# KC-decoder/Multimodal-Brain-Pattern-Identification_XAI

Measured on AMD Instinct MI355X. Metric: samples/sec train (multimodal SpectrogramCNN+EEGNet fusion, B=64/GPU, 4x128x256 spectro + 10000x19 EEG), higher is better.
Workload: dtype bf16

## Files before the change

include/brainxai.h:

```cpp
#ifndef BRAINXAI_H
#define BRAINXAI_H

#include <stddef.h>
#include <stdint.h>

#ifdef __cplusplus
extern "C" {
#endif

#define BX_VERSION 100

enum { BX_F32 = 0, BX_BF16 = 1 };
enum { BX_POOL_MAX = 0, BX_POOL_AVG = 1 };
enum { BX_OK = 0, BX_EINVAL = -1, BX_EDTYPE = -2, BX_EALIGN = -3, BX_EWORKSPACE = -4, BX_EHIP = -5,
       BX_EUNSUPPORTED = -6 };
enum { BX_ALGO_AUTO = 0, BX_ALGO_DIRECT = 1, BX_ALGO_MFMA = 2 };
enum { BX_EPI_RELU = 1, BX_EPI_MASK_BITS = 2 };

typedef void* bxStream;

int bx_version(void);
const char* bx_last_error_string(void);

int bx_nchw_to_nhwc(const float* src, void* dst, int B, int C, int H, int W, int Cp, int dtype, bxStream stream);
int bx_nhwc_to_nchw(const void* src, float* dst, int B, int C, int H, int W, int Cs, int dtype, bxStream stream);

int bx_conv3x3_pack(const float* w_oihw, float* packed_f32, void* packed_mfma, int Cout, int Cin,
                    int I_p, int O_p, int transpose_flip, bxStream stream);
size_t bx_conv3x3_packed_mfma_bytes(int I_p, int O_p);
size_t bx_conv3x3_packed_split_bytes(int I_p, int O_p);
int bx_conv3x3_pack_split(const float* w_oihw, void* packed_split, int Cout, int Cin, int I_p, int O_p, int transpose_flip,
                          bxStream stream);
typedef struct {
  const void* w_oihw;
  void* packed_mfma;
  int Cout, Cin, I_p, O_p, transpose_flip, block_begin;
} bxPackJob;
int bx_conv3x3_pack_many(const bxPackJob* jobs_device, int njobs, int total_blocks, bxStream stream);
int bx_conv3x3_pack_many_layout(const bxPackJob* jobs_device, int njobs, int total_blocks, const float* src_nchw,
                                void* dst_nhwc_bf16, int B, int C, int H, int W, int Cp, bxStream stream);
int bx_conv3x3_pack_layout_ex(const bxPackJob* jobs_device, int njobs, int total_blocks, const float* src_nchw,
                              const float* const* src_slot, void* dst_nhwc_bf16, int B, int C, int H, int W, int Cp, bxStream stream);
int bx_conv3x3_pack_many_step(const bxPackJob* jobs_device, int njobs, int total_blocks, const float* src_nchw,
                              void* dst_nhwc_bf16, int B, int C, int H, int W, int Cp, uint64_t* state_a, uint64_t* out_a,
                              uint64_t* state_b, uint64_t* out_b, bxStream stream);
int bx_conv3x3_pair_supported(int C0_p, int C1, int C2, int dtype);
int bx_conv3x3_pair(const void* x, const void* packed1_mfma, const float* bias1, const void* packed2_mfma, const float* bias2,
                    void* y1, void* y2, unsigned char* mask1, unsigned char* mask2, int B, int H, int W, int C0_p, int C1, int C2,
                    int dtype, bxStream stream);
int bx_conv3x3(const void* x, const float* packed_f32, const void* packed_mfma, const float* bias,
               const void* relu_mask_src, const void* addend, void* y,
               int B, int H, int W, int Ci, int Co, int dtype, int flags, int algo, bxStream stream);
size_t bx_conv3x3_wgrad_workspace(int B, int H, int W, int Ci_p, int Co, int dtype, int algo);
int bx_conv3x3_wgrad(const void* x, const void* dz, float* dw_oihw, float* dbias, int B, int H, int W,
                     int Cin, int Ci_p, int Co, int dtype, int algo, void* workspace, size_t workspace_bytes,
                     bxStream stream);
typedef struct {
  const void* partial; float* dw; float* db;
  int nsplit, Cin, Co, ma, nb, ztiles, nfrag4, valid;
} bxWgradPending;
int bx_conv3x3_wgrad_chained(const void* x, const void* dz, float* dw_oihw, float* dbias, int B, int H, int W, int Cin,
                             int Ci_p, int Co, int dtype, int algo, void* workspace, size_t workspace_bytes,
                             bxWgradPending* pending, bxStream stream);
int bx_conv3x3_wgrad_finish(bxWgradPending* pending, bxStream stream);
int bx_conv3x3_carry(const void* x, const float* packed_f32, const void* packed_mfma, const float* bias,
                     const void* relu_mask_src, const void* addend, void* y, int B, int H, int W, int Ci, int Co,
                     int dtype, int flags, int algo, bxWgradPending* pending, bxStream stream);
size_t bx_conv3x3_bwd_fused_workspace(int B, int H, int W, int with_w1);
int bx_conv3x3_bwd_fused(const void* dz, const void* xl, const void* packed_flip, void* dzo, const void* x0, float* dw, float* db,
                         float* dw0, float* db0, int B, int H, int W, int Cin0, void* workspace, size_t workspace_bytes,
                         bxWgradPending* pending, bxStream stream);

int bx_profile_next_conv3(void* ev_start, void* ev_stop);

typedef struct {
  int B, H, W;
  int Cin_p;
  int C;
  int pool;
  int training;
  float eps, momentum;
  float dropout_p;
  uint32_t salt;
  int dtype;
  uint32_t* sync;
  void* route;
} bxTailDesc;
size_t bx_block_tail_route_bytes(const bxTailDesc* d);
#define BX_TAIL_SYNC_WORDS 8192
#define BX_TAIL_SYNC_FWD 0
#define BX_TAIL_SYNC_BWD 4096
size_t bx_block_tail_workspace(const bxTailDesc* d);
int bx_block_tail_fwd(const bxTailDesc* d, const void* y3, const void* x, const float* w1x1, int Cin,
                      const float* b1x1, const float* bn_weight, const float* bn_bias,
                      float* running_mean, float* running_var, int64_t* num_batches_tracked,
                      const uint64_t* seed, void* pooled, void* out, float* save_mean, float* save_invstd,
                      void* workspace, size_t workspace_bytes, bxStream stream);
int bx_set_tree_max_rows(int rows);
int bx_set_tail_fold(int mask);
int bx_block_conv3_tail_fwd(const bxTailDesc* d, const void* y2, const void* w3_mfma, const float* b3, void* y3,
                            const void* x, const float* w1x1, int Cin, const float* b1x1, const float* bn_weight,
                            const float* bn_bias, float* running_mean, float* running_var, int64_t* num_batches_tracked,
                            const uint64_t* seed, void* pooled, void* out, float* save_mean, float* save_invstd,
                            void* workspace, size_t workspace_bytes, bxStream stream);
int bx_block_tail_bwd(const bxTailDesc* d, const void* dout, const void* y3, const void* x, const void* pooled,
                      const float* w1x1, int Cin, const float* bn_weight, const float* save_mean,
                      const float* save_invstd, const uint64_t* seed, void* dz3, void* dx_skip,
                      float* d_bn_weight, float* d_bn_bias, float* d_w1x1, float* d_b1x1,
                      void* workspace, size_t workspace_bytes, bxStream stream);
int bx_relu(const void* x, void* y, size_t n, int dtype, bxStream stream);

int bx_gap_fc_lsm_fwd(const void* feat, const float* w, const float* b, float* gap_out, float* logp,
                      int B, int HW, int C, int N, int dtype, bxStream stream);
int bx_gap_fc_lsm_bwd(const float* dlogp, const float* logp, const float* gap_out, const float* w,
                      void* dfeat, float* dw, float* db, int B, int HW, int C, int N, int dtype, bxStream stream);
int bx_linear_lsm_fwd(const float* x, const float* w, const float* b, float* logp, int B, int K, int N,
                      bxStream stream);
int bx_linear_lsm_bwd(const float* dlogp, const float* logp, const float* x, const float* w, float* dx,
                      float* dw, float* db, int B, int K, int N, bxStream stream);
int bx_fusion_head_fwd(const float* eeg_logp, const float* spec_logp, const float* w1, const float* b1,
                       const float* w2, const float* b2, float* hidden, float* logp, int B, int N, int Hd,
                       bxStream stream);
int bx_fusion_head_bwd(const float* dlogp, const float* logp, const float* hidden, const float* eeg_logp,
                       const float* spec_logp, const float* w1, const float* w2, float* d_eeg_logp,
// ... 151 lines not shown
```

multimodal-brain-pattern-identification_xai_amd/_lib.py:

```python
from __future__ import annotations

import ctypes as C
import os

HERE = os.path.dirname(os.path.abspath(__file__))
LIB_PATH = os.path.join(HERE, "libbrainxai.so")

BX_F32, BX_BF16 = 0, 1
BX_POOL_MAX, BX_POOL_AVG = 0, 1
BX_ALGO_AUTO, BX_ALGO_DIRECT, BX_ALGO_MFMA = 0, 1, 2
BX_EPI_RELU = 1
BX_EPI_MASK_BITS = 2
BX_TAIL_SYNC_WORDS = 8192
BX_EEG_CAM_CONV1, BX_EEG_CAM_DEPTHWISE, BX_EEG_CAM_SEPARABLE = 0, 1, 2

vp, i32, i64, u32, f32, sz = C.c_void_p, C.c_int, C.c_int64, C.c_uint32, C.c_float, C.c_size_t


class TailDesc(C.Structure):
    _fields_ = [("B", i32), ("H", i32), ("W", i32), ("Cin_p", i32), ("C", i32), ("pool", i32), ("training", i32),
                ("eps", f32), ("momentum", f32), ("dropout_p", f32), ("salt", u32), ("dtype", i32), ("sync", vp), ("route", vp)]


class EegDesc(C.Structure):
# ... 11 lines not shown
    _fields_ = [("B", i32), ("T2", i32), ("F2", i32), ("F3", i32), ("K3", i32), ("P3", i32), ("Hd", i32), ("N", i32), ("training", i32),
                ("eps", f32), ("momentum", f32), ("dropout_p", f32), ("salt", u32)]


class EegDeepParams(C.Structure):
    _fields_ = [(n, vp) for n in ("conv2_w", "bn4_w", "bn4_b", "bn4_rm", "bn4_rv", "bn4_nbt", "wq", "bq", "wk", "bk", "wv", "bv",
                                  "w1", "b1", "w2", "b2")]


class EegDeepGrads(C.Structure):
    _fields_ = [(n, vp) for n in ("conv2_w", "bn4_w", "bn4_b", "wq", "bq", "wk", "bk", "wv", "bv", "w1", "b1", "w2", "b2")]


class WgradPending(C.Structure):
    _fields_ = [("partial", vp), ("dw", vp), ("db", vp), ("nsplit", i32), ("Cin", i32), ("Co", i32), ("ma", i32), ("nb", i32),
                ("ztiles", i32), ("nfrag4", i32), ("valid", i32)]


class PackJob(C.Structure):
    _fields_ = [("w_oihw", vp), ("packed_mfma", vp), ("Cout", i32), ("Cin", i32), ("I_p", i32), ("O_p", i32),
                ("transpose_flip", i32), ("block_begin", i32)]


class EegGrads(C.Structure):
    _fields_ = [(n, vp) for n in ("conv1_w", "bn1_w", "bn1_b", "dw_w", "bn2_w", "bn2_b", "sep_w", "bn3_w", "bn3_b")]


P = C.POINTER
SIGNATURES = {
    "bx_version": (i32, []),
    "bx_last_error_string": (C.c_char_p, []),
    "bx_nchw_to_nhwc": (i32, [vp, vp, i32, i32, i32, i32, i32, i32, vp]),
    "bx_nhwc_to_nchw": (i32, [vp, vp, i32, i32, i32, i32, i32, i32, vp]),
    "bx_conv3x3_pack": (i32, [vp, vp, vp, i32, i32, i32, i32, i32, vp]),
    "bx_conv3x3_packed_mfma_bytes": (sz, [i32, i32]),
    "bx_conv3x3_packed_split_bytes": (sz, [i32, i32]),
    "bx_conv3x3_pack_split": (i32, [vp, vp, i32, i32, i32, i32, i32, vp]),
    "bx_conv3x3_pack_many": (i32, [vp, i32, i32, vp]),
    "bx_conv3x3_pack_many_layout": (i32, [vp, i32, i32, vp, vp, i32, i32, i32, i32, i32, vp]),
    "bx_conv3x3_pack_layout_ex": (i32, [vp, i32, i32, vp, vp, vp, i32, i32, i32, i32, i32, vp]),
    "bx_conv3x3_pair_supported": (i32, [i32, i32, i32, i32]),
    "bx_conv3x3_pair": (i32, [vp] * 9 + [i32] * 7 + [vp]),
    "bx_conv3x3_pack_many_step": (i32, [vp, i32, i32, vp, vp, i32, i32, i32, i32, i32, vp, vp, vp, vp, vp]),
    "bx_scale_dev": (i32, [vp, vp, vp, sz, vp]),
    "bx_abs": (i32, [vp, vp, sz, vp]),
    "bx_conv3x3": (i32, [vp, vp, vp, vp, vp, vp, vp, i32, i32, i32, i32, i32, i32, i32, i32, vp]),
    "bx_conv3x3_carry": (i32, [vp, vp, vp, vp, vp, vp, vp, i32, i32, i32, i32, i32, i32, i32, i32, P(WgradPending), vp]),
    "bx_conv3x3_wgrad_workspace": (sz, [i32, i32, i32, i32, i32, i32, i32]),
    "bx_conv3x3_wgrad": (i32, [vp, vp, vp, vp, i32, i32, i32, i32, i32, i32, i32, i32, vp, sz, vp]),
    "bx_conv3x3_wgrad_chained": (i32, [vp, vp, vp, vp, i32, i32, i32, i32, i32, i32, i32, i32, vp, sz, P(WgradPending), vp]),
    "bx_conv3x3_wgrad_finish": (i32, [P(WgradPending), vp]),
    "bx_conv3x3_bwd_fused_workspace": (sz, [i32, i32, i32, i32]),
    "bx_conv3x3_bwd_fused": (i32, [vp] * 9 + [i32] * 4 + [vp, sz, P(WgradPending), vp]),
    "bx_block_tail_workspace": (sz, [P(TailDesc)]),
    "bx_block_tail_fwd": (i32, [P(TailDesc), vp, vp, vp, i32, vp, vp, vp, vp, vp, vp, vp, vp, vp, vp, vp, vp, sz, vp]),
    "bx_set_tree_max_rows": (i32, [i32]),
    "bx_set_tail_fold": (i32, [i32]),
    "bx_block_tail_route_bytes": (sz, [vp]),
    "bx_block_conv3_tail_fwd": (i32, [P(TailDesc), vp, vp, vp, vp, vp, vp, i32, vp, vp, vp, vp, vp, vp, vp, vp, vp, vp, vp, vp, sz, vp]),
    "bx_block_tail_bwd": (i32, [P(TailDesc), vp, vp, vp, vp, vp, i32, vp, vp, vp, vp, vp, vp, vp, vp, vp, vp, vp, sz, vp]),
    "bx_relu": (i32, [vp, vp, sz, i32, vp]),
    "bx_gap_fc_lsm_fwd": (i32, [vp, vp, vp, vp, vp, i32, i32, i32, i32, i32, vp]),
    "bx_gap_fc_lsm_bwd": (i32, [vp, vp, vp, vp, vp, vp, vp, i32, i32, i32, i32, i32, vp]),
    "bx_linear_lsm_fwd": (i32, [vp, vp, vp, vp, i32, i32, i32, vp]),
    "bx_linear_lsm_bwd": (i32, [vp, vp, vp, vp, vp, vp, vp, i32, i32, i32, vp]),
    "bx_fusion_head_fwd": (i32, [vp, vp, vp, vp, vp, vp, vp, vp, i32, i32, i32, vp]),
    "bx_fusion_head_bwd": (i32, [vp] * 13 + [i32, i32, i32, vp]),
    "bx_mm_head_workspace": (sz, [i32, i32, i32]),
    "bx_mm_head_fwd": (i32, [vp] * 15 + [i32] * 7 + [vp]),
    "bx_mm_head_bwd": (i32, [vp] * 22 + [sz] + [i32] * 7 + [vp]),
    "bx_kldiv_fwd_bwd": (i32, [vp, vp, vp, vp, i32, i32, i32, f32, vp]),
    "bx_eeg_saved_bytes": (sz, [P(EegDesc)]),
    "bx_eeg_workspace": (sz, [P(EegDesc)]),
    "bx_eeg_features_fwd": (i32, [P(EegDesc), P(EegParams), vp, vp, vp, vp, vp, sz, vp]),
    "bx_eeg_features_bwd": (i32, [P(EegDesc), P(EegParams), vp, vp, vp, vp, P(EegGrads), vp, vp, sz, vp]),
    "bx_eeg_saved_layout": (i32, [P(EegDesc), P(sz), P(sz)]),
    "bx_eeg_gradcam_workspace": (sz, [P(EegDesc), i32, i32]),
    "bx_eeg_gradcam": (i32, [P(EegDesc), P(EegParams), vp, vp, vp, i32, i32, i32, vp, vp, vp, vp, sz, vp]),
    "bx_eeg_deep_saved_bytes": (sz, [P(EegDeepDesc)]),
    "bx_eeg_deep_workspace": (sz, [P(EegDeepDesc)]),
    "bx_eeg_deep_fwd": (i32, [P(EegDeepDesc), P(EegDeepParams), vp, vp, vp, vp, vp, vp, sz, vp]),
    "bx_eeg_deep_bwd": (i32, [P(EegDeepDesc), P(EegDeepParams), vp, vp, vp, vp, vp, P(EegDeepGrads), vp, vp, sz, vp]),
    "bx_attention_workspace": (sz, [i32]),
    "bx_attention_fwd": (i32, [vp] * 10 + [i32, i32, i32, vp]),
    "bx_attention_bwd": (i32, [vp] * 16 + [sz, i32, i32, i32, vp]),
    "bx_gradcam_reduce": (i32, [vp, vp, vp, vp, i32, i32, i32, i32, i32, i32, vp]),
    "bx_gradcam_head": (i32, [vp] * 12 + [i32] * 8 + [vp]),
    "bx_gradcam_head_sweep": (i32, [vp] * 4 + [i32] + [vp] * 8 + [i32] * 11 + [vp]),
    "bx_resize_bilinear": (i32, [vp, vp, i32, i32, i32, i32, i32, vp]),
    "bx_saliency_reduce": (i32, [vp, vp, i32, i32, i32, i32, f32, i32, vp]),
    "bx_axpby": (i32, [vp, vp, sz, f32, f32, vp]),
    "bx_mul": (i32, [vp, vp, vp, sz, vp]),
    "bx_ig_interpolate": (i32, [vp, vp, vp, vp, sz, i32, vp]),
    "bx_ig_accumulate": (i32, [vp, vp, vp, sz, i32, vp]),
    "bx_eeg_stack_iir": (i32, [vp, vp, vp, i32, i32, i32, i32, P(C.c_double), P(C.c_double), i32, i32, f32, f32, vp]),
    "bx_eeg_montage_workspace": (sz, [i32, i32, i32, i32]),
    "bx_eeg_montage_stack": (i32, [vp, vp, vp, vp, i32, i32, i32, i32, i32, P(C.c_double), P(C.c_double), i32, P(C.c_double), P(C.c_double),
                                   i32, f32, vp, vp, sz, vp]),
    "bx_spec_preprocess_workspace": (sz, [i32, i32, i32]),
    "bx_spec_preprocess": (i32, [vp, vp, vp, i32, i32, i32, i32, i32, i32, P(C.c_double), P(C.c_double), P(C.c_double), P(C.c_double),
                                 f32, vp, vp, sz, vp]),
    "bx_spec_regions_workspace": (sz, [i32]),
    "bx_spec_regions": (i32, [vp, vp, vp] + [i32] * 7 + [P(C.c_double), i32, P(C.c_double), i32, f32, vp, sz, vp]),
    "bx_adamw_step": (i32, [vp, vp, vp, vp, sz, f32, f32, f32, f32, f32, f32, vp, vp]),
    "bx_adamw_partials": (sz, [sz]),
    "bx_adamw_step_words": (sz, [sz]),
# ... 38 lines not shown
```

multimodal-brain-pattern-identification_xai_amd/csrc/conv3x3_mfma.hip:

```cpp
#include <stdlib.h>
#include "bx_common.h"
#include <string.h>

typedef __attribute__((ext_vector_type(8))) short bf16x8;
typedef __attribute__((ext_vector_type(4))) float f32x4;
typedef unsigned int u32x4 __attribute__((ext_vector_type(4)));
typedef unsigned int u32x2 __attribute__((ext_vector_type(2)));

static inline int mfma_ck(int Ci) { return Ci < 64 ? Ci : 64; }
static inline int mfma_ks(int ck) { return (9 * ck + 31) / 32; }

int bx_conv3x3_mfma_supported(int Ci, int Co, int dtype) {
  if (dtype != BX_BF16) return 0;
  if (!(Ci == 8 || Ci == 16 || Ci == 32 || (Ci >= 64 && Ci % 64 == 0))) return 0;
  return (Co >= 16 && Co % 16 == 0) || (Co == 8 && (Ci == 16 || Ci == 32));
}
static inline int mfma_ow(int O_p) { return O_p < 16 ? 16 : O_p; }
extern "C" size_t bx_conv3x3_packed_mfma_bytes(int I_p, int O_p) {
  if (!bx_conv3x3_mfma_supported(I_p, O_p, BX_BF16)) return 0;
  const int ck = mfma_ck(I_p);
  return (size_t)(I_p / ck) * mfma_ks(ck) * mfma_ow(O_p) * 32 * sizeof(bf16_t);
}

__global__ void k_pack_mfma(const float* __restrict__ w, bf16_t* __restrict__ wp, int Cout, int Cin, int I_p, int O_p, int tf,
// ... 2121 lines not shown
  constexpr int want_wgs = 512;
  const int want = want_wgs < p.ntiles ? want_wgs : p.ntiles;
  p.tps = (p.ntiles + want - 1) / want;
  p.nsplit = (p.ntiles + p.tps - 1) / p.tps;
  return p;
}
extern "C" size_t bx_conv3x3_bwd_fused_workspace(int B, int H, int W, int with_w1) {
  const FusedBwdPlan p = fused_bwd_plan(B, H, W);
  return (size_t)p.nsplit * (9 * 256 + 16) * sizeof(float) * (with_w1 ? 2 : 1);
}
extern "C" int bx_conv3x3_bwd_fused(const void* dz, const void* xl, const void* packed_flip, void* dzo, const void* x0, float* dw, float* db,
                                    float* dw0, float* db0, int B, int H, int W, int Cin0, void* ws, size_t ws_bytes, bxWgradPending* pending,
                                    bxStream stream) {
  hipStream_t s = (hipStream_t)stream;
  const bool w1 = x0 != nullptr;
  BX_REQUIRE(dz && xl && packed_flip && dw && db && ws && B > 0 && H > 0 && W > 0, "bx_conv3x3_bwd_fused: bad arguments");
  BX_REQUIRE(w1 ? (!dzo && dw0 && db0 && Cin0 > 0 && Cin0 <= 8) : (dzo && !dw0 && !db0),
             "bx_conv3x3_bwd_fused: either dzo (data gradient stored) or x0 with dw0 / db0 (conv1's weight gradient, 1..8 input channels)");
  BX_REQUIRE((size_t)B * H * W * 16 * 2 < ((size_t)1 << 31), "bx_conv3x3_bwd_fused: an activation tensor of 2 GiB or more is not supported");
  const FusedBwdPlan p = fused_bwd_plan(B, H, W);
  const size_t need = bx_conv3x3_bwd_fused_workspace(B, H, W, w1);
  BX_REQUIRE(ws_bytes >= need, "bx_conv3x3_bwd_fused: workspace %zu < %zu", ws_bytes, need);
  BX_REQUIRE(!pending || !pending->valid || pending->partial != ws, "bx_conv3x3_bwd_fused: the pending partials live in this call's workspace");
  WgradRedJob prev = {};
  int nred = 0;
  if (pending && pending->valid) { prev = wgrad_job_from(pending, true); nred = prev.nblocks; pending->valid = 0; }
  constexpr int IMG = 10 * 34 * 32;
  const size_t lds = w1 ? (size_t)3 * IMG + 8 * 32 * 32 : (size_t)2 * IMG;
  const uint32_t act_bytes = (uint32_t)((size_t)B * H * W * 16 * 2);
  float* part = (float*)ws;
  if (w1)
    hipLaunchKernelGGL((k_conv_mfma_bwd<true>), dim3((unsigned)(p.nsplit + nred)), dim3(256), lds, s, (const bf16_t*)dz, (const bf16_t*)xl,
                       (const bf16_t*)packed_flip, (const bf16_t*)x0, (bf16_t*)nullptr, part, H, W, p.tiles_x, p.tiles_y, p.ntiles, p.tps, p.nsplit,
                       act_bytes, prev, nred);
  else
    hipLaunchKernelGGL((k_conv_mfma_bwd<false>), dim3((unsigned)(p.nsplit + nred)), dim3(256), lds, s, (const bf16_t*)dz, (const bf16_t*)xl,
                       (const bf16_t*)packed_flip, (const bf16_t*)nullptr, (bf16_t*)dzo, part, H, W, p.tiles_x, p.tiles_y, p.ntiles, p.tps, p.nsplit,
                       act_bytes, prev, nred);
  BX_CHECK_LAUNCH("bx_conv3x3_bwd_fused");
  bxWgradPending cur = {};
  cur.partial = part; cur.dw = dw; cur.db = db; cur.nsplit = p.nsplit; cur.Cin = 16; cur.Co = 16; cur.ma = 1; cur.nb = 1;
  cur.ztiles = 1; cur.nfrag4 = 9 * 64; cur.valid = 1;
  if (!w1) {
    if (pending) { *pending = cur; return BX_OK; }
    return bx_wgrad_mfma_finish(&cur, s);
  }
  bxWgradPending cur0 = cur;
  cur0.partial = part + (size_t)p.nsplit * (9 * 256 + 16); cur0.dw = dw0; cur0.db = db0; cur0.Cin = Cin0;
  const WgradRedJob j1 = wgrad_job_from(&cur, false), j0 = wgrad_job_from(&cur0, false);
  hipLaunchKernelGGL(k_wgrad_reduce3, dim3((unsigned)(j1.nblocks + j0.nblocks)), dim3(256), 0, s, j1, j0);
  BX_CHECK_LAUNCH("bx_conv3x3_bwd_fused(reduce)");
  return BX_OK;
}
```

multimodal-brain-pattern-identification_xai_amd/ops.py:

```python
from __future__ import annotations

import ctypes as C
from types import SimpleNamespace

import torch

from . import _lib as L

CONV_ALGO = L.BX_ALGO_AUTO
WGRAD_ALGO = L.BX_ALGO_AUTO
CONV_PROFILE = None
import os as _os
OVERLAP_EEG = int(_os.environ.get("BX_OVERLAP_EEG", "1"))
OVERLAP_EEG_DDP = _os.environ.get("BX_OVERLAP_EEG_DDP", "0") == "1"


def overlap_eeg_now() -> bool:
    if CONV_PROFILE is not None or not (OVERLAP_EEG >= 2 or (OVERLAP_EEG == 1 and torch.cuda.is_current_stream_capturing())):
        return False
    import torch.distributed as dist
    return OVERLAP_EEG_DDP or not (dist.is_available() and dist.is_initialized())


def fork_eeg(device, *read_on_side):
# ... 387 lines not shown
def _wg_chain_state(device):
    key = device.index if device.index is not None else torch.cuda.current_device()
    st = _WG_CHAIN.get(key)
    if st is None:
        st = SimpleNamespace(pend=L.WgradPending(), ring=[None, None], slot=0, keep=None, stream=None, retired=[])
        _WG_CHAIN[key] = st
    return st


def wgrad_flush(device=None):
    for key, st in list(_WG_CHAIN.items()):
        if device is not None and key != (device.index if device.index is not None else torch.cuda.current_device()):
            continue
        if st.pend.valid:
            L.check(L.load().bx_conv3x3_wgrad_finish(C.byref(st.pend), st.stream), "bx_conv3x3_wgrad_finish")
        st.keep = None


def _wgrad(x, dz, w: torch.Tensor, b: torch.Tensor, chain: bool = False):
    lib = L.load()
    B, H, W, Cip = x.shape
    Co = dz.shape[3]
    dt = bx_dtype(x.dtype)
    algo = WGRAD_ALGO
    need = lib.bx_conv3x3_wgrad_workspace(B, H, W, Cip, Co, dt, algo)
    dw, db = new_grad(w), new_grad(b)
    if chain and WGRAD_CHAIN and algo != L.BX_ALGO_DIRECT:
        st = _wg_chain_state(x.device)
        if st.pend.valid and st.stream != _stream():
            wgrad_flush(x.device)
        buf = st.ring[st.slot]
        if buf is None or buf.numel() < need:
            if buf is not None:
                st.retired.append(buf)
            big = max([int(need), 1 << 20] + [b.numel() for b in st.ring if b is not None])
            buf = torch.empty(big, dtype=torch.uint8, device=x.device)
            st.ring[st.slot] = buf
        st.stream = _stream()
        with _Timed("wgrad", ("conv", B, H, W, Cip, Co)):
            L.check(lib.bx_conv3x3_wgrad_chained(_p(x), _p(dz), _p(dw), _p(db), B, H, W, w.shape[1], Cip, Co, dt, algo, _p(buf), buf.numel(),
                                                 C.byref(st.pend), st.stream), "bx_conv3x3_wgrad_chained")
        st.keep = (buf, dw, db)
        st.slot ^= 1
        return dw, db
    ws = workspace(need, x.device)
    with _Timed("wgrad", ("conv", B, H, W, Cip, Co)):
        L.check(lib.bx_conv3x3_wgrad(_p(x), _p(dz), _p(dw), _p(db), B, H, W, w.shape[1], Cip, Co, dt, algo, _p(ws), ws.numel(), _stream()),
                "bx_conv3x3_wgrad")
    return dw, db


def _bwd_fused(dz, xl, packed, w, b, x0, w0, b0):
    lib = L.load()
    B, H, W, _ = dz.shape
    st = _wg_chain_state(dz.device)
    if st.pend.valid and st.stream != _stream():
        wgrad_flush(dz.device)
    need = lib.bx_conv3x3_bwd_fused_workspace(B, H, W, 1 if x0 is not None else 0)
    buf = st.ring[st.slot]
    if buf is None or buf.numel() < need:
        if buf is not None:
            st.retired.append(buf)
        big = max([int(need), 1 << 20] + [t.numel() for t in st.ring if t is not None])
        buf = torch.empty(big, dtype=torch.uint8, device=dz.device)
        st.ring[st.slot] = buf
    st.stream = _stream()
    dw, db = new_grad(w), new_grad(b)
    dw0, db0 = (new_grad(w0), new_grad(b0)) if x0 is not None else (None, None)
    dzo = torch.empty_like(dz) if x0 is None else None
    if packed[1] is None or packed[4] != "bf16":
        raise RuntimeError("brainxai: the fused stage-1 backward needs the bf16 MFMA data-gradient operand")
    with _Timed("dgrad", ("conv", B, H, W, 16, 16)):
        L.check(lib.bx_conv3x3_bwd_fused(_p(dz), _p(xl), _p(packed[1]), _p(dzo), _p(x0), _p(dw), _p(db), _p(dw0), _p(db0), B, H, W,
                                         w0.shape[1], _p(buf), buf.numel(), C.byref(st.pend), st.stream), "bx_conv3x3_bwd_fused")
    if x0 is None:
        st.keep = (buf, dw, db)
        st.slot ^= 1
    else:
        st.keep = None
    return dw, db, dzo, (dw0, db0)


def _tail_desc(x, shape, dt, cfg, route=None) -> L.TailDesc:
    B, H, W, Cc = shape
    return L.TailDesc(B, H, W, x.shape[3], Cc, L.BX_POOL_MAX if cfg.pool == "max" else L.BX_POOL_AVG, 1 if cfg.training else 0,
                      cfg.eps, cfg.momentum, float(cfg.dropout_p), cfg.salt, bx_dtype(dt), _p(cfg.sync), _p(route))


class BlockFn(torch.autograd.Function):

    @staticmethod
    def forward(ctx, x, w1, b1, w2, b2, w3, b3, bnw, bnb, w11, b11, rm, rv, nbt, cfg):
        lib = L.load()
        dt = x.dtype
        ws_, bs_ = (w1, w2, w3), (b1, b2, b3)
        acts, pre = [x], None
        B, H, W, _ = x.shape
        Cc = w3.shape[0]
        fused = FUSE_POOL and dt == torch.bfloat16 and CONV_ALGO != L.BX_ALGO_DIRECT and cfg.preact != 3 and Cc >= 16
        packed3 = None
        first = 0
        masks = None
        fuse_bwd = False
        if (CONV_PAIR and dt == torch.bfloat16 and CONV_ALGO != L.BX_ALGO_DIRECT and cfg.preact not in (1, 2)
                and lib.bx_conv3x3_pair_supported(x.shape[3], w1.shape[0], w2.shape[0], bx_dtype(dt))):
            pk = []
            for k in range(2):
                packed = cfg.prepacked.get(cfg.pack_base + k, False) if cfg.prepacked is not None else None
                pk.append(packed if packed is not None else _pack(ws_[k], flip=False, dtype=dt))
            if pk[0][1] is not None and pk[1][1] is not None:
                need_y1 = cfg.keep is not None or (getattr(cfg, "grad_mode", True) and any(ctx.needs_input_grad[:11]))
                y1 = torch.empty(B, H, W, w1.shape[0], dtype=dt, device=x.device) if need_y1 else None
                y2 = torch.empty(B, H, W, w2.shape[0], dtype=dt, device=x.device)
                fuse_bwd = (need_y1 and cfg.keep is None and WGRAD_ALGO != L.BX_ALGO_DIRECT and x.shape[3] == 8
                            and tuple(w2.shape[:2]) == (16, 16) and tuple(w3.shape[:2]) == (16, 16) and any(ctx.needs_input_grad[1:11]))
                if need_y1 and MASK_BITS and w1.shape[0] <= 32 and not fuse_bwd:
                    masks = (torch.empty(B, H, W, w1.shape[0] // 4, dtype=torch.uint8, device=x.device),
                             torch.empty(B, H, W, w2.shape[0] // 4, dtype=torch.uint8, device=x.device))
                with _Timed("fwd", ("pair", B, H, W, x.shape[3], (w1.shape[0], w2.shape[0]))):
                    L.check(lib.bx_conv3x3_pair(_p(x), _p(pk[0][1]), _p(b1), _p(pk[1][1]), _p(b2), _p(y1), _p(y2),
                                                _p(masks[0]) if masks else None, _p(masks[1]) if masks else None, B, H, W, x.shape[3],
                                                w1.shape[0], w2.shape[0], bx_dtype(dt), _stream()), "bx_conv3x3_pair")
                acts += [y1 if y1 is not None else x.new_empty(0), y2]
                first = 2
        for k in range(first, 3):
            packed = cfg.prepacked.get(cfg.pack_base + k, False) if cfg.prepacked is not None else None
            if packed is None:
                packed = _pack(ws_[k], flip=False, dtype=dt)
            if k == 2 and fused and packed[1] is not None:
                packed3 = packed
                break
            if cfg.preact == k + 1:
                pre = _conv(acts[-1], packed, bs_[k], None, None, False, dt)
                y = torch.empty_like(pre)
                L.check(lib.bx_relu(_p(pre), _p(y), pre.numel(), bx_dtype(dt), _stream()), "bx_relu")
            else:
                y = _conv(acts[-1], packed, bs_[k], None, None, True, dt)
            acts.append(y)
        seed = None
        if cfg.training and cfg.dropout_p > 0:
            seed = cfg.seed if cfg.seed is not None else next_seed(x.device)
        pooled = torch.empty(B, H // 2, W // 2, Cc, dtype=dt, device=x.device)
        out = torch.empty_like(pooled)
        mean = torch.empty(Cc, dtype=torch.float32, device=x.device)
        invstd = torch.empty_like(mean)
        route = None
        if packed3 is not None:
            need_bwd = getattr(cfg, "grad_mode", True) and any(ctx.needs_input_grad[:11])
            use_route = TAIL_ROUTE and cfg.keep is None
            y3 = torch.empty(B, H, W, Cc, dtype=dt, device=x.device) if (cfg.keep is not None or (need_bwd and not use_route)) else None
            if need_bwd and use_route:
                route = torch.empty(B * (H // 2) * (W // 2) * Cc // 2, dtype=torch.uint8, device=x.device)
            desc = _tail_desc(x, (B, H, W, Cc), dt, cfg, route)
            ws = workspace(lib.bx_block_tail_workspace(C.byref(desc)), x.device)
            if CONV_PROFILE is not None:
                pe0, pe1 = torch.cuda.Event(enable_timing=True), torch.cuda.Event(enable_timing=True)
                pe0.record(); pe1.record()
                L.check(lib.bx_profile_next_conv3(pe0.cuda_event, pe1.cuda_event), "bx_profile_next_conv3")
                CONV_PROFILE.append(("fwd", pe0, pe1, ("conv3+pool", B, H, W, acts[2].shape[3], Cc)))
            L.check(lib.bx_block_conv3_tail_fwd(C.byref(desc), _p(acts[2]), _p(packed3[1]), _p(b3), _p(y3), _p(x), _p(w11), w11.shape[1], _p(b11),
                                                _p(bnw), _p(bnb), _p(rm), _p(rv), _p(nbt), _p(seed), _p(pooled), _p(out), _p(mean), _p(invstd),
                                                _p(ws), ws.numel(), _stream()), "bx_block_conv3_tail_fwd")
            acts.append(y3)
        else:
            y3 = acts[3]
            desc = _tail_desc(x, tuple(y3.shape), dt, cfg)
            ws = workspace(lib.bx_block_tail_workspace(C.byref(desc)), x.device)
            L.check(lib.bx_block_tail_fwd(C.byref(desc), _p(y3), _p(x), _p(w11), w11.shape[1], _p(b11), _p(bnw), _p(bnb), _p(rm), _p(rv), _p(nbt),
                                          _p(seed), _p(pooled), _p(out), _p(mean), _p(invstd), _p(ws), ws.numel(), _stream()), "bx_block_tail_fwd")
        ctx.cfg, ctx.desc, ctx.seed = cfg, desc, seed
        ctx.masks = masks
        ctx.fuse_bwd = fuse_bwd
        ctx.route, ctx.y3_shape = route, (B, H, W, Cc)
        ctx.save_for_backward(x, acts[1], acts[2], y3 if y3 is not None else x.new_empty(0), pooled, mean, invstd, w1, b1, w2, b2, w3, b3,
                              bnw, bnb, w11, b11)
        if pre is not None:
            cfg.capture["act"] = pre
        if cfg.keep is not None:
            cfg.keep["acts"] = (acts[1], acts[2], y3)
        return out

    @staticmethod
    def backward(ctx, dout):
        lib = L.load()
        x, y1, y2, y3, pooled, mean, invstd, w1, b1, w2, b2, w3, b3, bnw, bnb, w11, b11 = ctx.saved_tensors
        cfg, desc, seed = ctx.cfg, ctx.desc, ctx.seed
        dt = x.dtype
        need_dx = ctx.needs_input_grad[0]
        need_w = any(ctx.needs_input_grad[1:11])
        dout = dout.contiguous()
        dz3 = torch.empty(ctx.y3_shape, dtype=dt, device=x.device)
        if y3.numel() == 0:
            y3 = None
        dx_skip = torch.empty_like(x) if need_dx else None
        need_bn = ctx.needs_input_grad[7] or ctx.needs_input_grad[8]
        d_bnw, d_bnb = (new_grad(bnw), new_grad(bnb)) if need_bn else (torch.empty_like(bnw), torch.empty_like(bnb))
        d_w11, d_b11 = (new_grad(w11), new_grad(b11)) if need_w else (None, None)
        ws = workspace(lib.bx_block_tail_workspace(C.byref(desc)), x.device)
        L.check(lib.bx_block_tail_bwd(C.byref(desc), _p(dout), _p(y3), _p(x), _p(pooled), _p(w11), w11.shape[1], _p(bnw), _p(mean), _p(invstd),
                                      _p(seed), _p(dz3), _p(dx_skip), _p(d_bnw), _p(d_bnb), _p(d_w11), _p(d_b11), _p(ws), ws.numel(), _stream()),
                "bx_block_tail_bwd")
        if cfg.preact == 3:
            cfg.capture["grad"] = dz3
        acts = (x, y1, y2)
        wts = (w1, w2, w3)
        bss = (b1, b2, b3)
        grads_w, grads_b = [None] * 3, [None] * 3
        dz = dz3
        layers = (2, 1, 0)
        if ctx.fuse_bwd and need_w:
            for k in (2, 1):
                packed = cfg.prepacked.get(cfg.pack_base + k, True) if cfg.prepacked is not None else None
                w1_form = k == 1 and not need_dx
                grads_w[k], grads_b[k], dz, g0 = _bwd_fused(dz, acts[k], packed or _pack(wts[k], flip=True, dtype=dt), wts[k], bss[k],
                                                            x if w1_form else None, w1, b1)
            if w1_form:
                grads_w[0], grads_b[0] = g0
            layers = () if w1_form else (0,)
        for k in layers:
            if need_w:
                grads_w[k], grads_b[k] = _wgrad(acts[k], dz, wts[k], bss[k], chain=True)
            packed = cfg.prepacked.get(cfg.pack_base + k, True) if cfg.prepacked is not None else None
            if k > 0:
                mb = ctx.masks is not None and CONV_ALGO != L.BX_ALGO_DIRECT
                dz = _conv(dz, packed or _pack(wts[k], flip=True, dtype=dt), None, ctx.masks[k - 1] if mb else acts[k], None, False, dt,
                           mask_bits=mb)
                if cfg.preact == k:
                    cfg.capture["grad"] = dz
            elif need_dx:
                dz = _conv(dz, packed or _pack(wts[0], flip=True, dtype=dt), None, None, dx_skip, False, dt, carry=need_w)
        if need_w:
            wgrad_flush(x.device)
        dx = dz if need_dx else None
        if not need_bn:
            d_bnw = d_bnb = None
        return (dx, grads_w[0], grads_b[0], grads_w[1], grads_b[1], grads_w[2], grads_b[2], d_bnw, d_bnb, d_w11, d_b11,
                None, None, None, None)


class GapFcLsmFn(torch.autograd.Function):

    @staticmethod
    def forward(ctx, feat, w, b):
        B, H, W, Cc = feat.shape
        N = w.shape[0]
        gap = torch.empty(B, Cc, dtype=torch.float32, device=feat.device)
        logp = torch.empty(B, N, dtype=torch.float32, device=feat.device)
        L.check(L.load().bx_gap_fc_lsm_fwd(_p(feat), _p(w), _p(b), _p(gap), _p(logp), B, H * W, Cc, N, bx_dtype(feat.dtype), _stream()),
                "bx_gap_fc_lsm_fwd")
        ctx.shape, ctx.dt = (B, H, W, Cc), feat.dtype
        ctx.save_for_backward(gap, logp, w, b)
        return logp

    @staticmethod
    def backward(ctx, dlogp):
        gap, logp, w, b = ctx.saved_tensors
        B, H, W, Cc = ctx.shape
        N = w.shape[0]
        dfeat = torch.empty(B, H, W, Cc, dtype=ctx.dt, device=gap.device) if ctx.needs_input_grad[0] else None
        need_w = ctx.needs_input_grad[1] or ctx.needs_input_grad[2]
        dw, db = (new_grad(w), new_grad(b)) if need_w else (None, None)
        dlogp = dlogp.contiguous()
        L.check(L.load().bx_gap_fc_lsm_bwd(_p(dlogp), _p(logp), _p(gap), _p(w), _p(dfeat), _p(dw), _p(db), B, H * W, Cc, N,
                                           bx_dtype(ctx.dt), _stream()), "bx_gap_fc_lsm_bwd")
        return dfeat, dw, db

# ... 288 lines not shown
```

Baseline: 48380.

## Add fused dgrad+wgrad backward kernel for 32-channel conv3x3 stage

Adds an MFMA kernel that, for 32->32 conv3x3 layers, computes the data gradient (with ReLU masking from the saved activation) and accumulates the weight and bias gradient partials in the same pass over an LDS-staged tile. It also runs the previous layer's pending wgrad reduction in extra blocks. The Python path now routes the second-stage block (16->32->32->32, W>16) through this fused backward instead of separate dgrad and wgrad launches. This is meant to remove a second read of dz and activations plus launch overhead. In exchange the second stage no longer stores mask bits, and the kernel adds LDS and register pressure.

```diff
diff --git a/include/brainxai.h b/include/brainxai.h
--- a/include/brainxai.h
+++ b/include/brainxai.h
@@ -70,6 +70,9 @@
 int bx_conv3x3_bwd_fused(const void* dz, const void* xl, const void* packed_flip, void* dzo, const void* x0, float* dw, float* db,
                          float* dw0, float* db0, int B, int H, int W, int Cin0, void* workspace, size_t workspace_bytes,
                          bxWgradPending* pending, bxStream stream);
+size_t bx_conv3x3_bwd_fused32_workspace(int B, int H, int W);
+int bx_conv3x3_bwd_fused32(const void* dz, const void* xl, const void* packed_flip, void* dzo, float* dw, float* db, int B, int H, int W,
+                           int Cin, int Co, void* workspace, size_t workspace_bytes, bxWgradPending* pending, bxStream stream);
 
 int bx_profile_next_conv3(void* ev_start, void* ev_stop);
 
diff --git a/multimodal-brain-pattern-identification_xai_amd/_lib.py b/multimodal-brain-pattern-identification_xai_amd/_lib.py
--- a/multimodal-brain-pattern-identification_xai_amd/_lib.py
+++ b/multimodal-brain-pattern-identification_xai_amd/_lib.py
@@ -87,6 +87,8 @@
     "bx_conv3x3_wgrad_finish": (i32, [P(WgradPending), vp]),
     "bx_conv3x3_bwd_fused_workspace": (sz, [i32, i32, i32, i32]),
     "bx_conv3x3_bwd_fused": (i32, [vp] * 9 + [i32] * 4 + [vp, sz, P(WgradPending), vp]),
+    "bx_conv3x3_bwd_fused32_workspace": (sz, [i32, i32, i32]),
+    "bx_conv3x3_bwd_fused32": (i32, [vp] * 6 + [i32] * 5 + [vp, sz, P(WgradPending), vp]),
     "bx_block_tail_workspace": (sz, [P(TailDesc)]),
     "bx_block_tail_fwd": (i32, [P(TailDesc), vp, vp, vp, i32, vp, vp, vp, vp, vp, vp, vp, vp, vp, vp, vp, vp, sz, vp]),
     "bx_set_tree_max_rows": (i32, [i32]),
diff --git a/multimodal-brain-pattern-identification_xai_amd/csrc/conv3x3_mfma.hip b/multimodal-brain-pattern-identification_xai_amd/csrc/conv3x3_mfma.hip
--- a/multimodal-brain-pattern-identification_xai_amd/csrc/conv3x3_mfma.hip
+++ b/multimodal-brain-pattern-identification_xai_amd/csrc/conv3x3_mfma.hip
@@ -2197,3 +2197,209 @@
   BX_CHECK_LAUNCH("bx_conv3x3_bwd_fused(reduce)");
   return BX_OK;
 }
+
+__global__ __launch_bounds__(256, 2) void k_conv_mfma_bwd32(const bf16_t* __restrict__ dz, const bf16_t* __restrict__ xl, const bf16_t* __restrict__ wp,
+    bf16_t* __restrict__ dzo, float* __restrict__ partial, int H, int W, int tiles_x, int tiles_y, int ntiles, int tps, int nsplit,
+    uint32_t act_bytes, WgradRedJob red, int nred) {
+  constexpr int TH = 8, TW = 32, HWID = TW + 2, HH = TH + 2, RB = 64, KS = 9, MP = TH * TW / 64, TPR = TW / 16, NC = 2;
+  constexpr int NU = HH * HWID * 4, NR = (NU + 255) / 256;
+  constexpr int IMG = HH * HWID * RB;
+  constexpr int NT = 36, PER_SPLIT = NT * 256 + 32;
+  extern __shared__ __attribute__((aligned(16))) char lds[];
+  if ((int)blockIdx.x < nred) {
+    if ((int)blockIdx.x < red.nblocks) wgrad_reduce3_body(red, (int)blockIdx.x, reinterpret_cast<float4*>(lds));
+    return;
+  }
+  const int split = (int)blockIdx.x - nred;
+  char* xs = lds;
+  char* zs = lds + IMG;
+  const int wave = threadIdx.x >> 6, lane = threadIdx.x & 63, g = lane >> 4, li = lane & 15;
+  const int q = li >> 2, pc = li & 3;
+  const int m = wave >> 1, n = wave & 1;
+  const bool want_bias = m == 0;
+  const __amdgpu_buffer_rsrc_t zres = __builtin_amdgcn_make_buffer_rsrc((void*)dz, 0, act_bytes, 0x00020000);
+  const __amdgpu_buffer_rsrc_t xres = __builtin_amdgcn_make_buffer_rsrc((void*)xl, 0, act_bytes, 0x00020000);
+  const __amdgpu_buffer_rsrc_t yres = __builtin_amdgcn_make_buffer_rsrc((void*)dzo, 0, act_bytes, 0x00020000);
+  int hpy[NR], hpx[NR];
+  uint32_t hrel[NR];
+#pragma unroll
+  for (int k = 0; k < NR; ++k) {
+    const int u = threadIdx.x + k * 256;
+    const int p = u / 4, c = u % 4;
+    hpy[k] = u < NU ? p / HWID - 1 : -100000;
+    hpx[k] = p % HWID - 1;
+    hrel[k] = (uint32_t)(((p / HWID - 1) * W + (p % HWID - 1)) * 32 + c * 8) * 2u;
+  }
+  uint4 rz[NR], rx[NR];
+  auto fetch = [&](int tile) {
+    const int tx = tile % tiles_x, ty = (tile / tiles_x) % tiles_y, b = tile / (tiles_x * tiles_y);
+    const int y0 = ty * TH, xo = tx * TW;
+    const uint32_t pix0 = (uint32_t)((b * H + y0) * W + xo);
+#pragma unroll
+    for (int k = 0; k < NR; ++k) {
+      const bool ok = (unsigned)(y0 + hpy[k]) < (unsigned)H && (unsigned)(xo + hpx[k]) < (unsigned)W;
+      const uint32_t off = ok ? pix0 * 64u + hrel[k] : 0x80000000u;
+      const u32x4 v = __builtin_amdgcn_raw_buffer_load_b128(zres, off, 0, 0);
+      const u32x4 w = __builtin_amdgcn_raw_buffer_load_b128(xres, off, 0, 0);
+      rz[k] = make_uint4(v.x, v.y, v.z, v.w);
+      rx[k] = make_uint4(w.x, w.y, w.z, w.w);
+    }
+  };
+  int xbase[2], zbase[2];
+#pragma unroll
+  for (int h = 0; h < 2; ++h) {
+    const int c = 8 * g + 4 * h + q;
+    xbase[h] = c * RB + (((m ^ (c >> 3)) & 1) << 5) + pc * 8;
+    zbase[h] = (HWID + c + 1) * RB + (((n ^ ((c + 1) >> 2)) & 1) << 5) + pc * 8;
+  }
+  int xbase2;
+  {
+    const int c = 8 * g + q + 8;
+    xbase2 = c * RB + (((m ^ (c >> 3)) & 1) << 5) + pc * 8;
+  }
+  f32x4 aw[9];
+#pragma unroll
+  for (int t = 0; t < 9; ++t) aw[t] = (f32x4){0.f, 0.f, 0.f, 0.f};
+  float bsum = 0.f;
+  auto load_frags = [&](int ks, bf16x8 (&a)[9], bf16x8& bb) {
+    bb = tr_read8(zs, zbase[0] + ks * HWID * RB, zbase[1] + ks * HWID * RB);
+#pragma unroll
+    for (int dy = 0; dy < 3; ++dy) {
+      const int ro = (ks + dy) * HWID * RB;
+      const u32x2 p0 = __builtin_bit_cast(u32x2, __builtin_amdgcn_ds_read_tr16_b64_v4i16((lds_s16x4*)(xs + xbase[0] + ro)));
+      const u32x2 p1 = __builtin_bit_cast(u32x2, __builtin_amdgcn_ds_read_tr16_b64_v4i16((lds_s16x4*)(xs + xbase[1] + ro)));
+      const u32x2 p2 = __builtin_bit_cast(u32x2, __builtin_amdgcn_ds_read_tr16_b64_v4i16((lds_s16x4*)(xs + xbase2 + ro)));
+      const uint32_t d0 = p0.x, d1 = p0.y, d2 = p1.x, d3 = p1.y, d4 = p2.x;
+      a[dy * 3 + 0] = __builtin_bit_cast(bf16x8, (u32x4){d0, d1, d2, d3});
+      a[dy * 3 + 1] = __builtin_bit_cast(bf16x8, (u32x4){__builtin_amdgcn_alignbit(d1, d0, 16), __builtin_amdgcn_alignbit(d2, d1, 16),
+                                                         __builtin_amdgcn_alignbit(d3, d2, 16), __builtin_amdgcn_alignbit(d4, d3, 16)});
+      a[dy * 3 + 2] = __builtin_bit_cast(bf16x8, (u32x4){d1, d2, d3, d4});
+    }
+  };
+  auto mma = [&](const bf16x8 (&a)[9], const bf16x8& bb) {
+    if (want_bias) {
+#pragma unroll
+      for (int j = 0; j < 8; ++j) bsum += __uint_as_float(((uint32_t)(unsigned short)bb[j]) << 16);
+    }
+#pragma unroll
+    for (int tap = 0; tap < 9; ++tap) aw[tap] = __builtin_amdgcn_mfma_f32_16x16x32_bf16(a[tap], bb, aw[tap], 0, 0, 0);
+  };
+  const int t_begin = split * tps;
+  const int t_end = t_begin + tps < ntiles ? t_begin + tps : ntiles;
+  if (t_begin < t_end) fetch(t_begin);
+  for (int tile = t_begin; tile < t_end; ++tile) {
+    const int tx = tile % tiles_x, ty = (tile / tiles_x) % tiles_y, b = tile / (tiles_x * tiles_y);
+    const int y0 = ty * TH, xo = tx * TW;
+    __syncthreads();
+#pragma unroll
+    for (int k = 0; k < NR; ++k) {
+      const int u = threadIdx.x + k * 256, p = u >> 2, c = u & 3, px = p % HWID;
+      if (u < NU) {
+        *reinterpret_cast<uint4*>(xs + p * RB + ((((c >> 1) ^ (px >> 3)) & 1) << 5) + (c & 1) * 16) = rx[k];
+        *reinterpret_cast<uint4*>(zs + p * RB + ((((c >> 1) ^ (px >> 2)) & 1) << 5) + (c & 1) * 16) = rz[k];
+      }
+    }
+    __syncthreads();
+    if (tile + 1 < t_end) fetch(tile + 1);
+    f32x4 acc[MP][NC];
+#pragma unroll
+    for (int i = 0; i < MP; ++i)
+#pragma unroll
+      for (int nn = 0; nn < NC; ++nn) acc[i][nn] = (f32x4){0.f, 0.f, 0.f, 0.f};
+    const bf16_t* wt = wp;
+    asm volatile("" : "+s"(wt));
+    bf16x8 a[3][NC];
+    auto load_a = [&](int s, bf16x8 (&dst)[NC]) {
+#pragma unroll
+      for (int nn = 0; nn < NC; ++nn) dst[nn] = *reinterpret_cast<const bf16x8*>(wt + ((size_t)s * 32 + nn * 16 + li) * 32 + 8 * g);
+    };
+    load_a(0, a[0]);
+    load_a(1, a[1]);
+#pragma unroll
+    for (int s = 0; s < KS; ++s) {
+      if (s + 2 < KS) load_a(s + 2, a[(s + 2) % 3]);
+      __builtin_amdgcn_sched_barrier(0);
+      const int dy = s / 3, dx = s - 3 * dy;
+#pragma unroll
+      for (int i = 0; i < MP; ++i) {
+        const int t = wave * MP + i;
+        const int col = (t % TPR) * 16 + li + dx;
+        const int p = (t / TPR + dy) * HWID + col;
+        const bf16x8 bv = *reinterpret_cast<const bf16x8*>(zs + p * RB + 16 * (g ^ ((col >> 1) & 2)));
+#pragma unroll
+        for (int nn = 0; nn < NC; ++nn) acc[i][nn] = __builtin_amdgcn_mfma_f32_16x16x32_bf16(a[s % 3][nn], bv, acc[i][nn], 0, 0, 0);
+      }
+    }
+#pragma unroll
+    for (int i = 0; i < MP; ++i) {
+      const int t = wave * MP + i;
+      const int r = t / TPR, col = (t % TPR) * 16 + li;
+      const bool inb = y0 + r < H && xo + col < W;
+      const uint32_t orow = inb ? (uint32_t)((((b * H + y0 + r) * W + xo + col) * 32 + 4 * g) * 2) : 0x80000000u;
+#pragma unroll
+      for (int nn = 0; nn < NC; ++nn) {
+        const int hc = col + 1;
+        const u32x2 mk = *reinterpret_cast<const u32x2*>(xs + ((r + 1) * HWID + hc) * RB + (((nn ^ (hc >> 3)) & 1) << 5) + 8 * g);
+        const uint32_t mm[4] = {mk.x & 0xffffu, mk.x >> 16, mk.y & 0xffffu, mk.y >> 16};
+        float v[4] = {acc[i][nn][0] + 0.f, acc[i][nn][1] + 0.f, acc[i][nn][2] + 0.f, acc[i][nn][3] + 0.f};
+#pragma unroll
+        for (int j = 0; j < 4; ++j) v[j] = (mm[j] != 0u && mm[j] < 0x8000u) ? v[j] : 0.f;
+        const u32x2 out = {pack2bf(v[0], v[1]), pack2bf(v[2], v[3])};
+        __builtin_amdgcn_raw_buffer_store_b64(out, yres, inb ? orow + (uint32_t)(nn * 32) : 0x80000000u, 0, 0);
+      }
+    }
+    __builtin_amdgcn_sched_barrier(0);
+    {
+      bf16x8 a0[9], a1[9], b0, b1;
+      load_frags(0, a0, b0);
+#pragma unroll
+      for (int ks = 0; ks < TH; ks += 2) {
+        load_frags(ks + 1, a1, b1);
+        mma(a0, b0);
+        if (ks + 2 < TH) load_frags(ks + 2, a0, b0);
+        mma(a1, b1);
+      }
+    }
+  }
+  float* out = partial + (size_t)split * PER_SPLIT;
+  float4* out4 = reinterpret_cast<float4*>(out);
+#pragma unroll
+  for (int tap = 0; tap < 9; ++tap) out4[(tap * 4 + m * 2 + n) * 64 + lane] = make_float4(aw[tap][0], aw[tap][1], aw[tap][2], aw[tap][3]);
+  if (want_bias) {
+    float v = bsum;
+    v += __shfl_xor(v, 16, 64);
+    v += __shfl_xor(v, 32, 64);
+    if (lane < 16) out[NT * 256 + n * 16 + lane] = v;
+  }
+}
+
+extern "C" size_t bx_conv3x3_bwd_fused32_workspace(int B, int H, int W) {
+  const FusedBwdPlan p = fused_bwd_plan(B, H, W);
+  return (size_t)p.nsplit * (36 * 256 + 32) * sizeof(float);
+}
+extern "C" int bx_conv3x3_bwd_fused32(const void* dz, const void* xl, const void* packed_flip, void* dzo, float* dw, float* db, int B, int H,
+                                      int W, int Cin, int Co, void* ws, size_t ws_bytes, bxWgradPending* pending, bxStream stream) {
+  hipStream_t s = (hipStream_t)stream;
+  BX_REQUIRE(dz && xl && packed_flip && dzo && dw && db && ws && B > 0 && H > 0 && W > 0, "bx_conv3x3_bwd_fused32: bad arguments");
+  BX_REQUIRE(Cin == 32 && Co == 32, "bx_conv3x3_bwd_fused32: only 32 -> 32 layers (got %d -> %d)", Cin, Co);
+  BX_REQUIRE(W > 16, "bx_conv3x3_bwd_fused32: the map must be wider than 16 pixels (W = %d)", W);
+  BX_REQUIRE((size_t)B * H * W * 32 * 2 < ((size_t)1 << 31), "bx_conv3x3_bwd_fused32: an activation tensor of 2 GiB or more is not supported");
+  const FusedBwdPlan p = fused_bwd_plan(B, H, W);
+  const size_t need = bx_conv3x3_bwd_fused32_workspace(B, H, W);
+  BX_REQUIRE(ws_bytes >= need, "bx_conv3x3_bwd_fused32: workspace %zu < %zu", ws_bytes, need);
+  BX_REQUIRE(!pending || !pending->valid || pending->partial != ws, "bx_conv3x3_bwd_fused32: the pending partials live in this call's workspace");
+  WgradRedJob prev = {};
+  int nred = 0;
+  if (pending && pending->valid) { prev = wgrad_job_from(pending, true); nred = prev.nblocks; pending->valid = 0; }
+  constexpr size_t lds = (size_t)2 * 10 * 34 * 64;
+  const uint32_t act_bytes = (uint32_t)((size_t)B * H * W * 32 * 2);
+  float* part = (float*)ws;
+  hipLaunchKernelGGL(k_conv_mfma_bwd32, dim3((unsigned)(p.nsplit + nred)), dim3(256), lds, s, (const bf16_t*)dz, (const bf16_t*)xl,
+                     (const bf16_t*)packed_flip, (bf16_t*)dzo, part, H, W, p.tiles_x, p.tiles_y, p.ntiles, p.tps, p.nsplit, act_bytes, prev, nred);
+  BX_CHECK_LAUNCH("bx_conv3x3_bwd_fused32");
+  bxWgradPending cur = {};
+  cur.partial = part; cur.dw = dw; cur.db = db; cur.nsplit = p.nsplit; cur.Cin = 32; cur.Co = 32; cur.ma = 2; cur.nb = 2;
+  cur.ztiles = 1; cur.nfrag4 = 36 * 64; cur.valid = 1;
+  if (pending) { *pending = cur; return BX_OK; }
+  return bx_wgrad_mfma_finish(&cur, s);
+}
diff --git a/multimodal-brain-pattern-identification_xai_amd/ops.py b/multimodal-brain-pattern-identification_xai_amd/ops.py
--- a/multimodal-brain-pattern-identification_xai_amd/ops.py
+++ b/multimodal-brain-pattern-identification_xai_amd/ops.py
@@ -463,11 +463,12 @@
 
 def _bwd_fused(dz, xl, packed, w, b, x0, w0, b0):
     lib = L.load()
-    B, H, W, _ = dz.shape
+    B, H, W, Cz = dz.shape
     st = _wg_chain_state(dz.device)
     if st.pend.valid and st.stream != _stream():
         wgrad_flush(dz.device)
-    need = lib.bx_conv3x3_bwd_fused_workspace(B, H, W, 1 if x0 is not None else 0)
+    need = (lib.bx_conv3x3_bwd_fused_workspace(B, H, W, 1 if x0 is not None else 0) if Cz == 16
+            else lib.bx_conv3x3_bwd_fused32_workspace(B, H, W))
     buf = st.ring[st.slot]
     if buf is None or buf.numel() < need:
         if buf is not None:
@@ -480,10 +481,14 @@
     dw0, db0 = (new_grad(w0), new_grad(b0)) if x0 is not None else (None, None)
     dzo = torch.empty_like(dz) if x0 is None else None
     if packed[1] is None or packed[4] != "bf16":
-        raise RuntimeError("brainxai: the fused stage-1 backward needs the bf16 MFMA data-gradient operand")
-    with _Timed("dgrad", ("conv", B, H, W, 16, 16)):
-        L.check(lib.bx_conv3x3_bwd_fused(_p(dz), _p(xl), _p(packed[1]), _p(dzo), _p(x0), _p(dw), _p(db), _p(dw0), _p(db0), B, H, W,
-                                         w0.shape[1], _p(buf), buf.numel(), C.byref(st.pend), st.stream), "bx_conv3x3_bwd_fused")
+        raise RuntimeError("brainxai: the fused backward needs the bf16 MFMA data-gradient operand")
+    with _Timed("dgrad", ("conv", B, H, W, Cz, Cz)):
+        if Cz == 16:
+            L.check(lib.bx_conv3x3_bwd_fused(_p(dz), _p(xl), _p(packed[1]), _p(dzo), _p(x0), _p(dw), _p(db), _p(dw0), _p(db0), B, H, W,
+                                             w0.shape[1], _p(buf), buf.numel(), C.byref(st.pend), st.stream), "bx_conv3x3_bwd_fused")
+        else:
+            L.check(lib.bx_conv3x3_bwd_fused32(_p(dz), _p(xl), _p(packed[1]), _p(dzo), _p(dw), _p(db), B, H, W, xl.shape[3], Cz,
+                                               _p(buf), buf.numel(), C.byref(st.pend), st.stream), "bx_conv3x3_bwd_fused32")
     if x0 is None:
         st.keep = (buf, dw, db)
         st.slot ^= 1
@@ -523,8 +528,10 @@
                 need_y1 = cfg.keep is not None or (getattr(cfg, "grad_mode", True) and any(ctx.needs_input_grad[:11]))
                 y1 = torch.empty(B, H, W, w1.shape[0], dtype=dt, device=x.device) if need_y1 else None
                 y2 = torch.empty(B, H, W, w2.shape[0], dtype=dt, device=x.device)
-                fuse_bwd = (need_y1 and cfg.keep is None and WGRAD_ALGO != L.BX_ALGO_DIRECT and x.shape[3] == 8
-                            and tuple(w2.shape[:2]) == (16, 16) and tuple(w3.shape[:2]) == (16, 16) and any(ctx.needs_input_grad[1:11]))
+                fuse_bwd = (need_y1 and cfg.keep is None and WGRAD_ALGO != L.BX_ALGO_DIRECT and any(ctx.needs_input_grad[1:11])
+                            and ((x.shape[3] == 8 and tuple(w2.shape[:2]) == (16, 16) and tuple(w3.shape[:2]) == (16, 16))
+                                 or (x.shape[3] == 16 and W > 16 and tuple(w1.shape[:2]) == (32, 16) and tuple(w2.shape[:2]) == (32, 32)
+                                     and tuple(w3.shape[:2]) == (32, 32))))
                 if need_y1 and MASK_BITS and w1.shape[0] <= 32 and not fuse_bwd:
                     masks = (torch.empty(B, H, W, w1.shape[0] // 4, dtype=torch.uint8, device=x.device),
                              torch.empty(B, H, W, w2.shape[0] // 4, dtype=torch.uint8, device=x.device))
@@ -622,7 +629,7 @@
         if ctx.fuse_bwd and need_w:
             for k in (2, 1):
                 packed = cfg.prepacked.get(cfg.pack_base + k, True) if cfg.prepacked is not None else None
-                w1_form = k == 1 and not need_dx
+                w1_form = k == 1 and not need_dx and x.shape[3] == 8
                 grads_w[k], grads_b[k], dz, g0 = _bwd_fused(dz, acts[k], packed or _pack(wts[k], flip=True, dtype=dt), wts[k], bss[k],
                                                             x if w1_form else None, w1, b1)
             if w1_form:
```

Measured after the change: 49000 (median of 6 runs). 1.01x the previous value.
